# minyoungg/pix2latent

Measured on AMD Instinct MI355X. Metric: candidate-latent evals/sec (fwd+loss+bwd), BigGAN-256 pop=18, higher is better.
Workload: dtype f32 (fp32 tensors everywhere; convolutions >= 32x32 and the self-attention multiply on the 16-bit MFMA pipe with fp32-grade operand splits and fp32 accumulate: the 16x16 Winograd, direct and sub-pixel 3x3 kernels and the 1x1 kernels (4x4 layers included) on power-of-two scaled operands in 2 fp16 pie

## Files before the change

### include/p2l.h

```cpp
#ifndef P2L_H_
#define P2L_H_

#include <stddef.h>
#include <stdint.h>

#ifdef __cplusplus
extern "C" {
#endif

#define P2L_OK 0
#define P2L_EINVAL (-1)
#define P2L_ELAUNCH (-2)
#define P2L_EWS (-3)
#define P2L_EUNSUP (-4)

int p2l_version(void);
const char* p2l_strerror(int rc);
int p2l_last_hip_error(void);


enum { P2L_ACT_NONE = 0, P2L_ACT_RELU = 1, P2L_ACT_TANH = 2,
       P2L_ACT_LRELU_SQRT2 = 3  };
enum { P2L_POOL_NONE = 0, P2L_POOL_MAX = 1, P2L_POOL_SUM = 2 };
enum { P2L_PRO_NONE = 0, P2L_PRO_AFFINE_RELU = 1, P2L_PRO_AFFINE = 2 };
// ... 99 lines not shown

int p2l_pack_conv_weight(const float* w_oihw, int O, int I, int taps, int N_pad,
                         int K_pad, int transpose_flip, float* w_packed,
                         void* stream);

int p2l_pack_conv_weight_subpix(const float* w_oihw, int O, int I, int N_pad,
                                int K_pad, int transpose_flip, int mode,
                                float* w_packed, void* stream);

enum { P2L_WFMT_F32 = 0, P2L_WFMT_BF16X3 = 1, P2L_WFMT_BF16X3W = 2, P2L_WFMT_PW = 3,
       P2L_WFMT_BF16X3T = 4, P2L_WFMT_FLAG_PW = 0x10, P2L_WFMT_FLAG_THIN = 0x20,
       P2L_WFMT_FLAG_ATTN_GEMM = 0x40,
       P2L_WFMT_FLAG_NO_AMAX = 0x80
                                       };
int p2l_pack_conv_weight_bf3t(const float* w_oihw, int O, int I, int N_pad, int K_pad,
                              int transpose_flip, float* w_packed, void* stream);
int p2l_pack_conv_weight_pw(const float* w_oihw, int O, int I, int N_pad, int K_pad,
                            int transpose_flip, float* w_packed, void* stream);
size_t p2l_packed_weight_floats(int taps, int N_pad, int K_pad, int wfmt);
enum {
  P2L_FORM_AUTO = 0,
  P2L_FORM_NO_WINO = 1,
  P2L_FORM_WINO_ANY = 2,
  P2L_FORM_WINO_8X16 = 4,
  P2L_FORM_NO_PW = 8,
  P2L_FORM_NO_THIN = 16,
  P2L_FORM_WINO_BF3 = 32,
  P2L_FORM_WINO_H2_8X16 = 64,
  P2L_FORM_WINO_H2_16X16 = 128,
  P2L_FORM_NO_H2R = 256,
  P2L_FORM_H2R_SEQ_EPI = 512,
  P2L_FORM_NO_SP_SKIP = 1024,
  P2L_FORM_NO_SP_PAIR = 2048,
  P2L_FORM_SP_PAIR = 4096
};
int p2l_wino_split_factor(int H, int W, int Cin, int Cout);
int p2l_pack_conv_weight_bf3w(const float* w_oihw, int O, int I, int taps, int N_pad,
                              int K_pad, int transpose_flip, float* w_packed, void* stream);
int p2l_pack_conv_weight_bf3(const float* w_oihw, int O, int I, int taps, int N_pad,
                             int K_pad, int transpose_flip, float* w_packed, void* stream);
int p2l_pack_conv_weight_subpix_bf3(const float* w_oihw, int O, int I, int N_pad, int K_pad,
                                    int transpose_flip, int mode, float* w_packed,
                                    void* stream);
size_t p2l_packed_subpix_weight_floats(int N_pad, int K_pad, int wfmt);
int p2l_pack_conv_weight_subpix_h2(const float* w_oihw, int O, int I, int N_pad, int K_pad,
                                   int transpose_flip, int mode, float* w_packed, void* stream);

typedef struct P2LGemm {
  int32_t batch, M, N, K;
  int32_t lda, ldb, ldc;
  int64_t stride_a, stride_b, stride_c;
  int32_t a_kmajor, b_kmajor;
  float alpha;
  int32_t accumulate;
} P2LGemm;
int p2l_gemm(const P2LGemm* d, const float* A, const float* B, float* C,
             void* stream);
size_t p2l_gemm_ws_bytes(const P2LGemm* d);
int p2l_gemm_ws(const P2LGemm* d, const float* A, const float* B, float* C, void* ws,
                size_t ws_bytes, void* stream);

typedef struct P2LAttn {
  int32_t B, Nq, Nk, d, dv;
} P2LAttn;
int p2l_attn_supported(const P2LAttn* d);
size_t p2l_attn_fwd_ws_bytes(const P2LAttn* d);
int p2l_attn_fwd(const P2LAttn* d, const float* q, const float* k, const float* v, float* out,
                 float* lse, void* ws, size_t ws_bytes, void* stream);
// ... 384 lines not shown
```

### pix2latent_amd/_native.py

```python
import ctypes as C
import os

import torch

_HERE = os.path.dirname(os.path.abspath(__file__))
LIB_PATH = os.environ.get('P2L_LIB_PATH') or os.path.join(_HERE, 'libp2l_hip.so')

c_float_p = C.c_void_p


class P2LConv(C.Structure):
    _fields_ = [('B', C.c_int32), ('H', C.c_int32), ('W', C.c_int32),
                ('Cin', C.c_int32), ('Cout', C.c_int32), ('taps', C.c_int32),
                ('ups', C.c_int32), ('x_ld', C.c_int32), ('pro', C.c_int32),
                ('pro_bstride', C.c_int32), ('alpha', C.c_float), ('act', C.c_int32),
                ('pool', C.c_int32), ('y_ld', C.c_int32), ('yp_ld', C.c_int32),
                ('n_store', C.c_int32), ('res_ld', C.c_int32), ('res_ups', C.c_int32),
                ('mask_ld', C.c_int32), ('splitk', C.c_int32), ('ext', C.c_int32),
                ('wfmt', C.c_int32), ('form', C.c_int32), ('algo_flops', C.c_double),
                ('w_floats', C.c_int64)]


class P2LAmax(C.Structure):
    _fields_ = [('out', C.c_void_p), ('outp', C.c_void_p), ('in_', C.c_void_p), ('in_n', C.c_int32),
# ... 111 lines not shown
class P2LProfTotals(C.Structure):
    _fields_ = [('size', C.c_uint32), ('count', C.c_int32 * 2), ('reserved0', C.c_int32),
                ('flops', C.c_double * 2), ('ms', C.c_double * 2), ('bytes', C.c_double * 2),
                ('exec_flops', C.c_double * 2), ('mfma_flops', C.c_double * 2),
                ('write_bytes', C.c_double * 2),
                ('fam_count', C.c_int32 * 8), ('fam_ms', C.c_double * 8), ('fam_flops', C.c_double * 8),
                ('fam_mfma_flops', C.c_double * 8), ('fam_bytes', C.c_double * 8)]


PROF_FAMILIES = {0: 'other (exact-fp32 / bf16x3 direct, 8x16 Winograd)', 1: 'wino16s_conv_kernel<.., H2>',
                 2: 'conv_h2_kernel<9, ..>', 3: 'conv_h2_kernel<4, ..>', 4: 'conv_thinin/thinout_kernel',
                 5: 'pw_h2_kernel / pw_conv_kernel', 6: 'conv_h2r_kernel<..>'}


def prof_totals():
    t = P2LProfTotals()
    t.size = C.sizeof(P2LProfTotals)
    check(lib().p2l_prof_totals(C.byref(t)), 'p2l_prof_totals')
    return t


prof_end = prof_totals


ACT_NONE, ACT_RELU, ACT_TANH, ACT_LRELU_SQRT2 = 0, 1, 2, 3
WFMT_F32, WFMT_BF16X3, WFMT_BF16X3W, WFMT_PW, WFMT_BF16X3T = 0, 1, 2, 3, 4
WFMT_FLAG_PW, WFMT_FLAG_THIN, WFMT_FLAG_ATTN_GEMM, WFMT_FLAG_NO_AMAX = 0x10, 0x20, 0x40, 0x80
FORM_AUTO, FORM_NO_WINO, FORM_WINO_ANY, FORM_WINO_8X16, FORM_NO_PW, FORM_NO_THIN, FORM_WINO_BF3 = 0, 1, 2, 4, 8, 16, 32
FORM_WINO_H2_8X16, FORM_WINO_H2_16X16 = 64, 128
FORM_H2R_SEQ_EPI = 512
FORM_NO_SP_SKIP = 1024
FORM_NO_SP_PAIR = 2048
FORM_SP_PAIR = 4096
FORM_NO_H2R = 256


def default_wfmt():
    v = os.environ.get('P2L_CONV_WFMT', 'bf16x3').lower()
    if v in ('f32', 'fp32', '0'):
        return WFMT_F32
    if v in ('bf16x3-direct', 'bf3d', '1'):
        return WFMT_BF16X3
    if v in ('bf16x3', 'bf3', 'bf16x3w', '2'):
        return WFMT_BF16X3W
    raise ValueError('P2L_CONV_WFMT=%r (expected f32, bf16x3 or bf16x3-direct)' % v)


def default_thin():
    return os.environ.get('P2L_THIN', '1') != '0' and default_wfmt() != WFMT_F32


def default_attn_gemm():
    return os.environ.get('P2L_ATTN', '1') == '0'


def default_no_amax():
    return os.environ.get('P2L_AMAX', '1') == '0'


def default_pw():
    return os.environ.get('P2L_PW', '1') != '0' and default_wfmt() != WFMT_F32


def pack_conv_weight(src, taps, n_pad, k_pad, flip, wfmt, subpix_mode=None):
    L = lib()
    O, I = src.shape[0], src.shape[1]
# ... 9 lines not shown
    if subpix_mode is not None:
        dst = torch.empty(L.p2l_packed_subpix_weight_floats(n_pad, k_pad, wfmt), device=src.device,
                          dtype=torch.float32)
        fn = {WFMT_F32: L.p2l_pack_conv_weight_subpix,
              WFMT_BF16X3W: L.p2l_pack_conv_weight_subpix_h2}.get(wfmt, L.p2l_pack_conv_weight_subpix_bf3)
        check(fn(ptr(src), O, I, n_pad, k_pad, int(flip), int(subpix_mode), ptr(dst), stream()),
              'p2l_pack_conv_weight_subpix')
        return dst
    n = L.p2l_packed_weight_floats(taps, n_pad, k_pad, wfmt)
    dst = torch.empty(n, device=src.device, dtype=torch.float32)
    if wfmt == WFMT_BF16X3T:
        check(L.p2l_pack_conv_weight_bf3t(ptr(src), O, I, n_pad, k_pad, int(flip), ptr(dst), stream()),
              'p2l_pack_conv_weight_bf3t')
        return dst
    fn = {WFMT_F32: L.p2l_pack_conv_weight, WFMT_BF16X3: L.p2l_pack_conv_weight_bf3,
          WFMT_BF16X3W: L.p2l_pack_conv_weight_bf3w}[wfmt]
    check(fn(ptr(src), O, I, taps, n_pad, k_pad, int(flip), ptr(dst), stream()),
          'p2l_pack_conv_weight')
    return dst
def pack_gconv_weight(src, taps, n_pad, k_pad, flip):
    L = lib()
    src = src.detach().float().contiguous()
    dst = torch.empty(taps * n_pad * k_pad, device=src.device, dtype=torch.float32)
    check(L.p2l_pack_gconv_weight(ptr(src), src.shape[0], src.shape[1], taps, n_pad, k_pad, int(flip), ptr(dst),
                                  stream()), 'p2l_pack_gconv_weight')
    return dst


POOL_NONE, POOL_MAX, POOL_SUM = 0, 1, 2
PRO_NONE, PRO_AFFINE_RELU, PRO_AFFINE = 0, 1, 2

EXPORTS = [
    'p2l_version', 'p2l_strerror', 'p2l_last_hip_error',
    'p2l_conv_workspace_bytes', 'p2l_conv_amax_slots', 'p2l_selftest_amaxreg', 'p2l_conv_suggest_splitk', 'p2l_conv_fwd', 'p2l_conv_fwd_ex',
    'p2l_pack_conv_weight', 'p2l_pack_conv_weight_subpix', 'p2l_pack_conv_weight_bf3',
    'p2l_pack_conv_weight_bf3w', 'p2l_packed_weight_floats', 
    'p2l_pack_conv_weight_bf3t',
    'p2l_pack_conv_weight_pw', 'p2l_adam_step_dev',
    'p2l_attn_supported', 'p2l_attn_fwd_ws_bytes', 'p2l_attn_fwd', 'p2l_attn_bwd_dv_ws_bytes',
    'p2l_attn_bwd_dv', 'p2l_attn_bwd_qk_ws_bytes', 'p2l_attn_bwd_qk',
    'p2l_pack_conv_weight_subpix_bf3', 'p2l_pack_conv_weight_subpix_h2', 'p2l_packed_subpix_weight_floats', 'p2l_gemm', 'p2l_gemm_ws_bytes', 'p2l_gemm_ws', 'p2l_linear_fwd', 'p2l_linear_bwd',
    'p2l_cbn_fold_fwd', 'p2l_cbn_fold_bwd', 'p2l_affine_relu_bwd_nblk',
    'p2l_affine_relu_bwd', 'p2l_softmax_fwd', 'p2l_softmax_bwd', 'p2l_maxpool2_bwd', 'p2l_maxpool2_bwd_amax', 'p2l_maxpool2_bwd_amax_slots',
    'p2l_relu_mask', 'p2l_nchw3_to_nhwc16', 'p2l_nhwc16_to_nchw3', 'p2l_tanh_bwd16',
    'p2l_weight_sum', 'p2l_weight_map', 'p2l_l1_loss_nblk', 'p2l_l1_loss_fwd',
    'p2l_l1_loss_bwd', 'p2l_lpips_normalize', 'p2l_lpips_tap_nblk', 'p2l_lpips_tap_fwd',
    'p2l_lpips_tap_bwd', 'p2l_lpips_tap_pool_bwd', 'p2l_bilinear_adjoint', 'p2l_reduce_rows', 'p2l_adam_step',
    'p2l_clamp', 'p2l_affine_grid_sample', 'p2l_affine_grid_sample_bwd', 'p2l_affine_grid_sample_bwd_ws_bytes', 'p2l_vec_scale_div', 'p2l_concat2', 'p2l_split2',
    'p2l_biggan_ws_bytes', 'p2l_biggan_fwd', 'p2l_biggan_bwd', 'p2l_biggan_ws_lookup',
    'p2l_loss_cache_floats', 'p2l_projloss_ws_bytes', 'p2l_projloss_ws_lookup', 'p2l_projloss_prepare',
    'p2l_projloss_fwd', 'p2l_projloss_bwd', 'p2l_mfma_probe', 'p2l_prof_begin', 'p2l_prof_totals', 'p2l_prof_step', 'p2l_prof_dump', 'p2l_wino_split_factor', 'p2l_linear_fwd_ld', 'p2l_linear_bwd_ld', 'p2l_scale_bwd',
    'p2l_sg2_pixelnorm_fwd', 'p2l_sg2_pixelnorm_bwd', 'p2l_sg2_bias_lrelu_fwd', 'p2l_sg2_lrelu_bwd',
    'p2l_sg2_demod_fwd', 'p2l_sg2_demod_bwd', 'p2l_sg2_blur_fwd', 'p2l_sg2_act_bwd_nblk',
    'p2l_sg2_styled_act_bwd', 'p2l_sg2_blur_bwd', 'p2l_sg2_rgb_up_fwd', 'p2l_sg2_rgb_up_bwd',
    'p2l_sg2_clamp16_fwd', 'p2l_sg2_clamp16_bwd', 'p2l_broadcast_rows', 'p2l_add_inplace',
    'p2l_sg2_ws_bytes', 'p2l_sg2_ws_lookup', 'p2l_sg2_synthesis_fwd', 'p2l_sg2_synthesis_bwd', 'p2l_sg2_mapping_fwd',
    'p2l_sg2_mapping_bwd', 'p2l_conv_arb_fusable', 'p2l_conv_arb_nblk',
    'p2l_conv_dgrad_arb', 'p2l_conv_arb_split_fusable', 'p2l_conv_arb_nblk_ws',
    'p2l_conv_dgrad_arb_ws', 'p2l_arb_finish', 'p2l_arb_defer_begin', 'p2l_arb_defer_flush',
    'p2l_arb_defer_cancel',
    'p2l_gconv_fwd', 'p2l_maxpool3s2_fwd', 'p2l_maxpool3s2_bwd', 'p2l_conv1_dgrad',
    'p2l_alex_cache_floats', 'p2l_alexloss_ws_bytes', 'p2l_alexloss_prepare', 'p2l_alexloss_fwd',
    'p2l_alexloss_bwd',
    'p2l_pack_gconv_weight', 'p2l_sqz_cache_floats', 'p2l_sqzloss_ws_bytes', 'p2l_sqzloss_prepare', 'p2l_sqzloss_fwd',
    'p2l_sqzloss_bwd', 'p2l_sqzloss_ws_lookup',
    'p2l_sg2_blur_fwd_amax', 'p2l_sg2_styled_act_bwd_amax', 'p2l_sg2_blur_bwd_amax', 'p2l_sg2_noise_relayout',
    'p2l_sg2_rows_defer_begin', 'p2l_sg2_rows_defer_flush', 'p2l_sg2_rows_defer_cancel',
# ... 90 lines not shown
```

### pix2latent_amd/csrc/p2l_conv.hip

```cpp
#include "p2l_conv_k.h"

#include <cstdlib>
#include <cstring>
#include <cstddef>
#include <array>
#include <atomic>
#include <cstdio>
#include <mutex>
#include <string>
#include <vector>

using namespace p2lconv;

namespace {

struct ConvProf {
  std::atomic<bool> on{false};
  int n = 0;
  std::vector<hipEvent_t> ev;
  std::vector<double> flops;
  std::vector<double> xflops;
  std::vector<int> nprod;
  std::vector<double> bytes;
  std::vector<double> wbytes;
// ... 964 lines not shown
static bool direct_h2r(const P2LConv* d) {
  if ((d->form & P2L_FORM_NO_H2R) || !direct_h2(d)) return false;
  if (!p2l_h2r_shape(d->taps, d->ups, d->H, d->W, d->Cin, d->Cout, d->x_ld)) return false;
  return d->H * d->W >= 128 && direct_split(d) <= 1;
}


static int subpix_bwd_split(const P2LConv* d) {
  if (d->ups != 3 || !d->ext || !direct_h2(d)) return 1;
  ConvK k{};
  if (choose_tile(d, k) != P2L_OK || k.partial) return 1;
  const long hw = (long)(d->H >> 1) * (d->W >> 1);
  int s = p2f((long)d->Cin * 16 / 128);
  const int g = p2f(524288L / (hw * d->Cout > 0 ? hw * d->Cout : 1));
  if (g < s) s = g;
  const int cap = hw >= 256 ? 4 : 8;
  if (s > cap) s = cap;
  const int nchunks = 4 * (d->Cin / 16);
  while (s > 1 && nchunks / s < 8) s >>= 1;
  return s <= 2 ? 1 : s;
}

extern "C" int p2l_conv_suggest_splitk(const P2LConv* d) {
  ConvK k{};
  if (d && d->ups == 3 && d->ext) return subpix_bwd_split(d);
  if (!d || d->ups >= 2) return 1;
  if (choose_tile(d, k) == P2L_OK && wino_split(d) > 1 && !(d->form & P2L_FORM_WINO_ANY) &&
      (d->H / 8) * (d->W / 16) * (d->Cout / 64) < 64)
    return wino_split(d);
  if (choose_tile(d, k) != P2L_OK || k.partial || wino_shape(d) || pw_any(d)) return 1;
  return direct_split(d);
}

static bool wino_h2(const P2LConv* d) {
  return wino_shape(d) && d->H % 16 == 0 && d->W % 16 == 0 &&
         !(d->form & (P2L_FORM_WINO_8X16 | P2L_FORM_WINO_BF3));
}
static int effective_splitk(const P2LConv* d);
static bool finish_v4_ok(const P2LConv* d) {
#ifdef P2L_AB_SCALAR_FINISH
  return false;
#endif
  return d->n_store % 4 == 0 && d->Cout % 4 == 0 && d->y_ld % 4 == 0 && d->yp_ld % 4 == 0 &&
         d->res_ld % 4 == 0 && d->mask_ld % 4 == 0;
}
extern "C" int p2l_conv_amax_slots(const P2LConv* d) {
  if (!d) return 0;
  if (wino_shape(d)) {
    if (d->H % 16 || d->W % 16 || (d->form & P2L_FORM_WINO_8X16)) return 0;
    if (d->splitk > 1 && wino_split(d) == d->splitk) {
      const int per_image = (d->H / 2) * (d->W / 2) * (d->n_store / 4);
      return (per_image % 64 == 0 && d->n_store % 4 == 0) ? per_image / 64 : 0;
    }
    return (d->H / 16) * (d->W / 16) * (d->Cout / 64) * 8;
  }
  if (d->ups == 3 && effective_splitk(d) > 1) return 0;
  if (effective_splitk(d) > 1) {
    const int per_image = (d->H / 2) * (d->W / 2) * (finish_v4_ok(d) ? d->n_store / 4 : d->n_store);
    return (per_image % 64 == 0) ? per_image / 64 : 0;
  }
  ConvK k{};
  if (choose_tile(d, k) != P2L_OK || k.tb_log != 0 || k.partial) return 0;
  const int tm = thin_shape(d);
  if (tm >= 0) {
    const bool geom = k.tw_log == 4 && k.th_log == 3;
    return (tm == 1 && geom) ? k.tiles_x * k.tiles_y * 4 : 0;
// ... 719 lines not shown
```

### pix2latent_amd/csrc/p2l_conv_k.h

```cpp
#pragma once
#include "p2l_common.h"

namespace p2lconv {

struct ConvK {
  const float* x;
  const float* w;
  const float* bias;
  const float* pro_s;
  const float* pro_t;
  const float* res;
  const float* mask;
  float* y;
  float* yp;
  float* ws;
  int B, H, W, Cin, Cout;
  int x_ld, y_ld, yp_ld, res_ld, mask_ld, n_store;
  int pro_bstride;
  float alpha;
  int act, pool, res_ups, ups;
  int nchunks, chunks_per_split, splitk;
  int tw_log, th_log, tb_log;
  int tiles_x_log, tiles_y_log;
  int n_mtiles, n_ntiles;
// ... 343 lines not shown
      if (k.amax_out != nullptr) k.amax_out[slot] = m;
      if (k.amax_outp != nullptr) k.amax_outp[slot] = mp;
    }
  }
}


}

int p2l_pw_launch(const p2lconv::ConvK& k, int pro, hipStream_t st);

size_t p2l_thin_weight_floats(int N_pad, int K_pad);
int p2l_thin_mode(int N_pad, int K_pad);
int p2l_thin_pack(const float* w_oihw, int O, int I, int N_pad, int K_pad, int flip, float* dst,
                  hipStream_t st);
int p2l_thinin_launch(const p2lconv::ConvK& k, int pro, hipStream_t st);
int p2l_thinout_launch(const p2lconv::ConvK& k, int pro, hipStream_t st);

extern "C" size_t p2l_wino_weight_floats(int N_pad, int K_pad);
extern "C" int p2l_wino_weight_ok(int N_pad, int K_pad);
extern "C" int p2l_wino_split_factor(int H, int W, int Cin, int Cout);
extern "C" size_t p2l_wino_h2_weight_floats(int N_pad, int K_pad);
extern "C" size_t p2l_pw_h2_weight_floats(int N_pad, int K_pad);
int p2l_pw_pack_h2(const float* w_oihw, int O, int I, int N_pad, int K_pad, int flip, float* dst, hipStream_t st);
int p2l_wino_pack(const float* w_oihw, int O, int I, int N_pad, int K_pad, int transpose_flip,
                  float* dst, hipStream_t st);
int p2l_wino_launch(const p2lconv::ConvK& k, int pro, hipStream_t st);
int p2l_amax_launch(const p2lconv::ConvK& k, int pro, hipStream_t st);

size_t p2l_h2_weight_floats(int N_pad, int K_pad, int subpix);
int p2l_h2_pack(const float* w_oihw, int O, int I, int N_pad, int K_pad, int flip, int mode, float* dst,
                hipStream_t st);
int p2l_h2_launch(const p2lconv::ConvK& k, int pro, int taps, int bn, bool small, hipStream_t st);

bool p2l_h2r_shape(int taps, int ups, int H, int W, int Cin, int Cout, int x_ld);
bool p2l_h2r_takes(const p2lconv::ConvK& k);
int p2l_h2r_launch(const p2lconv::ConvK& k, int pro, hipStream_t st);
```

### pix2latent_amd/csrc/p2l_h2.hip

```cpp
#include "p2l_conv_k.h"

#include <atomic>
#include <type_traits>

using namespace p2lconv;

namespace {

#ifndef P2L_H2_ABL
#define P2L_H2_ABL 0
#endif

__device__ __forceinline__ int h2c(int c, int row) { return c ^ ((row >> 2) & 3) ^ (((row >> 1) & 1) << 1); }

#define P2L_WAIT(VM, LGKM) __builtin_amdgcn_s_waitcnt(((VM) & 15) | (7 << 4) | ((LGKM) << 8) | (((VM) >> 4) << 14))

template <int TAPS, int BN, int A_ITERS, int PRO, bool SKIP = false>
__global__ __launch_bounds__(256, 2) void conv_h2_kernel(const ConvK k) {
  constexpr bool SUBPIX = (TAPS == 4 || TAPS == 8);
  constexpr int NP = (TAPS == 8) ? 2 : 1;
  constexpr int NT = BN / 32;
  constexpr int B_ITEMS = TAPS * BN * 4;
  constexpr int B_ITERS = (B_ITEMS + 255) / 256;
  constexpr int SL = SUBPIX ? 16 : TAPS;
  constexpr int T0 = (TAPS == 4) ? 2 : 4;
  constexpr int NU = TAPS * NT, U0 = T0 * NT;
  constexpr int H0 = U0 * 128;
  static_assert(H0 % 256 == 0, "half 0 must be whole DMA instructions");
  constexpr int NH1_MIN = (B_ITEMS - H0) / 256;
  constexpr bool S_UNI = (A_ITERS == 3);
  constexpr int S_ITERS = S_UNI ? 1 : A_ITERS;
  constexpr int NA_LD = A_ITERS + ((PRO != P2L_PRO_NONE) ? 2 * S_ITERS : 0);

  extern __shared__ __attribute__((aligned(16))) float smem[];

  const int tid = threadIdx.x;
  const int lane = tid & 63, wave = tid >> 6;
  const int l31 = lane & 31, lhi = lane >> 5;

  const int TW = 1 << k.tw_log, TH = 1 << k.th_log, TB = 1 << k.tb_log;
  const int HW_ = TW + 2, HH_ = TH + 2;
  const int HP = k.hp;
  const int a_rows = TB * HH_ * HW_;
  const int a_rows_lds = TB * HH_ * HP;
  char* As = reinterpret_cast<char*>(smem);
  char* Bs = As + (size_t)a_rows_lds * 64;
  const int main_floats = max(a_rows_lds * 16 + TAPS * BN * 16, 4 * 32 * (BN + 4));
  float* scl = smem + main_floats;

  const int swz = xcd_remap(blockIdx.x, gridDim.x);
  const int mt = swz / k.n_ntiles, nt = swz - mt * k.n_ntiles;
  const int tiles_per_image = k.tiles_x * k.tiles_y;
  const int bt = mt / tiles_per_image;
  const int tile_in_image = mt - bt * tiles_per_image;
  const int ty = tile_in_image / k.tiles_x, tx = tile_in_image - ty * k.tiles_x;
  const int n0 = nt * BN;
  const int y0 = ty << k.th_log, x0 = tx << k.tw_log, b0 = bt << k.tb_log;

  const bool sp_fwd = SUBPIX && (TAPS == 8 || k.sp_mode == 1);
  const bool sp_bwd = (TAPS == 4) && k.sp_mode == 2;
  const int z = sp_fwd ? 0 : blockIdx.y;
  const int ph_y = sp_fwd ? (TAPS == 8 ? (int)blockIdx.y : (int)(blockIdx.y >> 1)) : 0;
  const int ph_x = (sp_fwd && TAPS == 4) ? (int)(blockIdx.y & 1) : 0;
  const int c_begin = z * k.chunks_per_split;
  const int c_end = min(k.nchunks, c_begin + k.chunks_per_split);

  const int av = tid & 3;
  int a_goff[A_ITERS];
  int a_soff[A_ITERS];
  int a_row[A_ITERS];
  float a_xs[S_ITERS];
  int a_tb[S_ITERS];
  unsigned a_valid = 0;
#pragma unroll
  for (int it = 0; it < A_ITERS; ++it) {
    const int p = (tid + 256 * it) >> 2;
    a_goff[it] = 0;
    a_soff[it] = 0;
    a_row[it] = -1;
    if (it < S_ITERS) { a_xs[it] = 1.f; a_tb[it] = 0; }
// ... 30 lines not shown
        a_extra = ((cls >> 1) * k.ibW + (cls & 1)) * k.x_ld;
      } else {
        wslab = (ph_y * 2 + ph_x) * 4;
      }
    }
  };
  int b_goff[B_ITERS];
#pragma unroll
  for (int it = 0; it < B_ITERS; ++it) {
    const int jj = tid + 256 * it;
    const int u = jj >> 7, within = jj & 127;
    const int tap = u / NT, j = u - tap * NT;
    b_goff[it] = ((j * SL + tap) * 32) * 16 + within * 4;
  }
  auto dma_b = [&](int c, auto half_c) {
    constexpr int half = decltype(half_c)::value;
    int cc, wslab, a_extra;
    geom(c, cc, wslab, a_extra);
    const float* base = k.w + ((((size_t)cc * (k.Cout >> 5) + (n0 >> 5)) * SL + wslab) * 32) * 16;
#pragma unroll
    for (int it = 0; it < B_ITERS; ++it) {
      if ((half == 0 && 256 * it >= H0) || (half == 1 && 256 * (it + 1) <= H0)) continue;
      const int jj = tid + 256 * it;
      if (jj < B_ITEMS) {
        const float* src = base + b_goff[it];
        if (SUBPIX && SKIP) {
          unsigned lv;
          if (TAPS == 8) { const unsigned my = ph_y ? 0x3u : 0xFu; lv = my | ((my & 0x5u) << 4); }
          else if (sp_fwd) lv = (ph_y ? 0x3u : 0xFu) & (ph_x ? 0x5u : 0xFu);
          else { const int cls = c / k.sp_ncc; lv = ((cls >> 1) ? 0xCu : 0xFu) & ((cls & 1) ? 0xAu : 0xFu); }
          const int tap = (jj >> 7) / NT;
          if (!((lv >> tap) & 1u)) src = base;
        }
        const unsigned lds_wave_base = __builtin_amdgcn_readfirstlane(
            (unsigned)(size_t)(__attribute__((address_space(3))) char*)(Bs + (size_t)(jj - lane) * 16));
        asm volatile("s_mov_b32 m0, %1\n\ts_nop 0\n\tglobal_load_lds_dwordx4 %0, off"
                     :: "v"(src), "s"(lds_wave_base) : "memory");
      }
    }
  };
  auto load_a = [&](int c) {
    int cc, wslab, a_extra;
    geom(c, cc, wslab, a_extra);
#pragma unroll
    for (int it = 0; it < A_ITERS; ++it) {
      xr[it] = *reinterpret_cast<const f32x4*>(k.x + (size_t)(a_goff[it] + a_extra) + cc * 16);
      if (PRO != P2L_PRO_NONE && it < S_ITERS) {
        const int so = S_UNI ? s_uni : a_soff[it];
        sr[it] = *reinterpret_cast<const f32x4*>(k.pro_s + so + cc * 16);
        tr[it] = *reinterpret_cast<const f32x4*>(k.pro_t + so + cc * 16);
      }
    }
  };
  auto write_a = [&]() {
#pragma unroll
    for (int it = 0; it < A_ITERS; ++it) {
      if (a_row[it] >= 0) {
        f32x4 v = xr[it];
        if (PRO != P2L_PRO_NONE) {
          v = v * sr[S_UNI ? 0 : it] + tr[S_UNI ? 0 : it];
          if (PRO == P2L_PRO_AFFINE_RELU) {
            v.x = fmaxf(v.x, 0.f); v.y = fmaxf(v.y, 0.f);
            v.z = fmaxf(v.z, 0.f); v.w = fmaxf(v.w, 0.f);
          }
        }
        if (!((a_valid >> it) & 1u)) v = f32x4{0.f, 0.f, 0.f, 0.f};
        v = v * a_xs[S_UNI ? 0 : it];
        const h16x4 h = __builtin_convertvector(v, h16x4);
        const f32x4 w = __builtin_convertvector(h, f32x4);
        const h16x4 m = __builtin_convertvector(v - w, h16x4);
        const int row = a_row[it];
        char* rb = As + row * 64 + (av & 1) * 8;
        *reinterpret_cast<h16x4*>(rb + h2c(av >> 1, row) * 16) = h;
        *reinterpret_cast<h16x4*>(rb + h2c(2 + (av >> 1), row) * 16) = m;
      }
    }
  };

  int a_row0;
  {
    const int i = wave * 32 + l31;
    const int Q = i >> 2, s = i & 3;
    const int qx = Q & ((TW >> 1) - 1);
    const int qy = (Q >> (k.tw_log - 1)) & ((TH >> 1) - 1);
    const int tb = Q >> (k.tw_log + k.th_log - 2);
    a_row0 = (tb * HH_ + 2 * qy + (s >> 1)) * HP + 2 * qx + (s & 1);
  }
  const int b_h = l31 * 64 + h2c(lhi, l31) * 16, b_m = l31 * 64 + h2c(2 + lhi, l31) * 16;

  f32x16 acc[NP * NT];
#pragma unroll
  for (int j = 0; j < NP * NT; ++j)
#pragma unroll
    for (int r = 0; r < 16; ++r) acc[j][r] = 0.f;

  using H0c = std::integral_constant<int, 0>;
  using H1c = std::integral_constant<int, 1>;
  if (c_begin < c_end) {
    dma_b(c_begin, H0c{});
    dma_b(c_begin, H1c{});
    load_a(c_begin);
  }
  {
    float sw, inv_w;
    h2_scales(__builtin_amdgcn_readfirstlane(k.w_tail[0]), sw, inv_w);
    const int step = (TB == 1) ? 256 : 64, me = (TB == 1) ? tid : lane;
    for (int t = (TB == 1) ? 0 : wave; t < TB; t += 4) {
      const int b = b0 + t;
      float a = 0.f, ms = 0.f, mtt = 0.f;
      if (b < k.B) {
        if (k.amax_in != nullptr) {
          for (int i = me; i < k.amax_in_n; i += step) a = fmaxf(a, k.amax_in[(size_t)b * k.amax_in_n + i]);
          if (PRO != P2L_PRO_NONE && !k.amax_in_applied) {
            const f32x4* ps = reinterpret_cast<const f32x4*>(k.pro_s + (size_t)b * k.pro_bstride);
            const f32x4* pt = reinterpret_cast<const f32x4*>(k.pro_t + (size_t)b * k.pro_bstride);
            for (int c = me; c < (k.Cin >> 2); c += step) {
              const f32x4 s4 = ps[c], t4 = pt[c];
              ms = fmaxf(fmaxf(ms, fmaxf(fabsf(s4.x), fabsf(s4.y))), fmaxf(fabsf(s4.z), fabsf(s4.w)));
              mtt = fmaxf(fmaxf(mtt, fmaxf(fabsf(t4.x), fabsf(t4.y))), fmaxf(fabsf(t4.z), fabsf(t4.w)));
            }
          }
        } else if (me < 64) {
          a = k.amax[b * 64 + me];
        }
      }
#pragma unroll
      for (int o = 1; o < 64; o <<= 1) {
        a = fmaxf(a, __shfl_xor(a, o, 64));
        if (PRO != P2L_PRO_NONE) { ms = fmaxf(ms, __shfl_xor(ms, o, 64)); mtt = fmaxf(mtt, __shfl_xor(mtt, o, 64)); }
      }
      if (TB == 1) {
        if (lane == 0) { smem[wave * 4] = a; smem[wave * 4 + 1] = ms; smem[wave * 4 + 2] = mtt; }
        __syncthreads();
        a = fmaxf(fmaxf(smem[0], smem[4]), fmaxf(smem[8], smem[12]));
        ms = fmaxf(fmaxf(smem[1], smem[5]), fmaxf(smem[9], smem[13]));
        mtt = fmaxf(fmaxf(smem[2], smem[6]), fmaxf(smem[10], smem[14]));
      }
      if (PRO != P2L_PRO_NONE && k.amax_in != nullptr) a = (k.amax_in_applied ? a : ms * a + mtt) * 1.001f;
      float xs, inv_x;
      h2_scales(__builtin_bit_cast(unsigned, a), xs, inv_x);
      if ((TB == 1) ? (tid == 0) : (lane == 0)) { scl[2 * t] = xs; scl[2 * t + 1] = inv_x * inv_w; }
      if (TB == 1) break;
    }
    __syncthreads();
  }

  if (S_UNI) {
    a_xs[0] = scl[0];
  } else {
#pragma unroll
    for (int it = 0; it < S_ITERS; ++it) a_xs[it] = scl[2 * a_tb[it]];
  }
  if (c_begin < c_end) {
    write_a();
    __builtin_amdgcn_sched_barrier(0);
    if (c_begin + 1 < c_end) load_a(c_begin + 1);
  }
  __builtin_amdgcn_sched_barrier(0);
  P2L_WAIT(NA_LD, 0);
  __builtin_amdgcn_s_barrier();

  for (int c = c_begin; c < c_end; ++c) {
    const bool more = (c + 1 < c_end);
    int win_row = 0;
    if (SUBPIX) {
      int oy = ph_y, ox = ph_x;
      if (sp_bwd) {
        const int cls = c / k.sp_ncc;
        oy = 1 - (cls >> 1);
        ox = 1 - (cls & 1);
      }
      win_row = oy * HP + ox;
    }
    unsigned live = 0xFFu;
    if (SUBPIX && SKIP) {
      if (TAPS == 8) {
        const unsigned my = ph_y ? 0x3u : 0xFu;
        live = my | ((my & 0x5u) << 4);
      } else if (sp_fwd) {
        live = (ph_y ? 0x3u : 0xFu) & (ph_x ? 0x5u : 0xFu);
      } else {
        const int cls = c / k.sp_ncc;
        live = ((cls >> 1) ? 0xCu : 0xFu) & ((cls & 1) ? 0xAu : 0xFu);
      }
    }
    h16x8 af[2][2], bq[2][2];
    auto lda = [&](int tap, h16x8 (&a)[2]) {
      const int dy = (TAPS == 9) ? tap / 3 : ((tap & 3) >> 1);
      const int dx = (TAPS == 9) ? tap - dy * 3 : (tap & 1);
      const int arow = a_row0 + win_row + dy * HP + dx + ((TAPS == 8) ? (tap >> 2) : 0);
      const char* ar = As + arow * 64;
      a[0] = *reinterpret_cast<const h16x8*>(ar + h2c(lhi, arow) * 16);
      a[1] = *reinterpret_cast<const h16x8*>(ar + h2c(2 + lhi, arow) * 16);
    };
    auto ldb = [&](int u, h16x8 (&b)[2]) {
      const char* br = Bs + u * (32 * 64);
      b[0] = *reinterpret_cast<const h16x8*>(br + b_h);
      b[1] = *reinterpret_cast<const h16x8*>(br + b_m);
    };
    lda(0, af[0]);
    ldb(0, bq[0]);
#pragma unroll
    for (int u = 0; u < NU; ++u) {
      const int tap = u / NT, j = u - tap * NT;
      if (u == U0) {
        if (more) P2L_WAIT(NA_LD, 0); else P2L_WAIT(0, 0);
        if (!(P2L_H2_ABL & 16)) __builtin_amdgcn_s_barrier();
        if (more && !(P2L_H2_ABL & 4)) dma_b(c + 1, H0c{});
        if (j == 0) lda(tap, af[tap & 1]);
        ldb(u, bq[u & 1]);
      }
      if (u + 1 < NU && u + 1 != U0) {
        const int tn = (u + 1) / NT, jn = (u + 1) - tn * NT;
        if (!(SUBPIX && SKIP) || ((live >> tn) & 1u)) {
          if (jn == 0) lda(tn, af[tn & 1]);
          ldb(u + 1, bq[(u + 1) & 1]);
        }
      }
      __builtin_amdgcn_sched_barrier(0);
      const h16x8 (&a)[2] = af[tap & 1];
      const h16x8 (&b)[2] = bq[u & 1];
      if (SUBPIX && SKIP && !((live >> tap) & 1u)) continue;
      const int ja = (TAPS == 8) ? (tap >> 2) * NT + j : j;
      if (!(P2L_H2_ABL & 8)) {
      acc[ja] = __builtin_amdgcn_mfma_f32_32x32x16_f16(a[1], b[0], acc[ja], 0, 0, 0);
      acc[ja] = __builtin_amdgcn_mfma_f32_32x32x16_f16(a[0], b[1], acc[ja], 0, 0, 0);
      acc[ja] = __builtin_amdgcn_mfma_f32_32x32x16_f16(a[0], b[0], acc[ja], 0, 0, 0);
      } else { acc[ja][0] += (float)a[0][0] * (float)b[0][0]; }
      __builtin_amdgcn_sched_barrier(0);
    }
    P2L_WAIT(63, 0);
    if (!(P2L_H2_ABL & 16)) __builtin_amdgcn_s_barrier();
    if (more) {
      if (!(P2L_H2_ABL & 1)) write_a();
      __builtin_amdgcn_sched_barrier(0);
      const bool more2 = (c + 2 < c_end);
      if (!(P2L_H2_ABL & 4)) dma_b(c + 1, H1c{});
      __builtin_amdgcn_sched_barrier(0);
      if (more2 && !(P2L_H2_ABL & 2)) load_a(c + 2);
      __builtin_amdgcn_sched_barrier(0);
      if (more2) P2L_WAIT(NA_LD + NH1_MIN, 0); else P2L_WAIT(NH1_MIN, 0);
    } else {
      P2L_WAIT(63, 0);
    }
    if (!(P2L_H2_ABL & 16)) __builtin_amdgcn_s_barrier();
  }

  if (S_UNI) {
    const float os = scl[1];
#pragma unroll
    for (int j = 0; j < NP * NT; ++j)
#pragma unroll
      for (int r = 0; r < 16; ++r) acc[j][r] *= os;
  } else {
#pragma unroll
    for (int g = 0; g < 4; ++g) {
      const int Q = wave * 8 + 2 * g + lhi;
      const float os = scl[2 * (Q >> (k.tw_log + k.th_log - 2)) + 1];
#pragma unroll
      for (int j = 0; j < NP * NT; ++j)
#pragma unroll
        for (int s = 0; s < 4; ++s) acc[j][4 * g + s] *= os;
    }
  }

  if (k.splitk > 1) {
    const size_t mtot = (size_t)k.B * k.H * k.W;
#pragma unroll
    for (int g = 0; g < 4; ++g) {
      const int Q = wave * 8 + 2 * g + lhi;
      const int qx = Q & ((TW >> 1) - 1);
      const int qy = (Q >> (k.tw_log - 1)) & ((TH >> 1) - 1);
      const int b = b0 + (Q >> (k.tw_log + k.th_log - 2));
      if (b >= k.B) continue;
      const size_t pix0 = ((size_t)b * k.H + y0 + 2 * qy) * k.W + x0 + 2 * qx;
#pragma unroll
      for (int j = 0; j < NT; ++j) {
        float* wp = k.ws + ((size_t)z * mtot + pix0) * k.Cout + n0 + j * 32 + l31;
        wp[0] = acc[j][g * 4 + 0];
        wp[k.Cout] = acc[j][g * 4 + 1];
        wp[(size_t)k.W * k.Cout] = acc[j][g * 4 + 2];
        wp[(size_t)(k.W + 1) * k.Cout] = acc[j][g * 4 + 3];
      }
    }
  } else {
    __syncthreads();
    if (!(P2L_H2_ABL & 32) || acc[0][0] == 12345.678f) {
      if (TAPS == 8) {
#pragma unroll
        for (int p = 0; p < NP; ++p) {
          if (p) __syncthreads();
          epilogue_vec<NT>(k, reinterpret_cast<f32x16 (&)[NT]>(acc[p * NT]), smem, wave, lane, b0, y0, x0, n0,
                           tile_in_image, 1, ph_y, p);
        }
      } else {
        epilogue_vec<NT>(k, reinterpret_cast<f32x16 (&)[NT]>(acc[0]), smem, wave, lane, b0, y0, x0, n0, tile_in_image,
                         sp_fwd ? 1 : 0, ph_y, ph_x);
      }
    }
// ... 67 lines not shown
                        : src[((size_t)n * I + c) * 9 + dy * 3 + dx];
      }
    }
    const float x = v * scale;
    const _Float16 h = (_Float16)x;
    ph[e] = h; pm[e] = (_Float16)(x - (float)h);
  }
  char* rb = reinterpret_cast<char*>(dst) +
             ((((size_t)q * (N_pad >> 5) + tile) * n_slabs + slab) * 32 + row) * 64;
  *reinterpret_cast<h16x8*>(rb + h2c(kh, row) * 16) = ph;
  *reinterpret_cast<h16x8*>(rb + h2c(2 + kh, row) * 16) = pm;
}

}

size_t p2l_h2_weight_floats(int N_pad, int K_pad, int subpix) {
  return (size_t)N_pad * K_pad * (subpix ? 16 : 9) + 4;
}
int p2l_h2_pack(const float* w_oihw, int O, int I, int N_pad, int K_pad, int flip, int mode, float* dst,
                hipStream_t st) {
  const int n_slabs = mode < 0 ? 9 : 16;
  unsigned* tail = reinterpret_cast<unsigned*>(dst + (size_t)N_pad * K_pad * n_slabs);
  if (hipMemsetAsync(tail, 0, 16, st) != hipSuccess) return P2L_ELAUNCH;
  const size_t nw = (size_t)O * I * 9;
  hipLaunchKernelGGL(h2_wmax_kernel, dim3((unsigned)(cdiv(nw, 256) < 256 ? cdiv(nw, 256) : 256)), dim3(256), 0, st,
                     w_oihw, nw, tail);
  if (mode >= 0) hipLaunchKernelGGL(h2_tail_x4_kernel, dim3(1), dim3(1), 0, st, tail);
  const size_t total = (size_t)(K_pad >> 4) * (N_pad >> 5) * n_slabs * 32 * 2;
  hipLaunchKernelGGL(h2_pack_kernel, dim3(cdiv(total, 256)), dim3(256), 0, st, w_oihw, dst, O, I, N_pad, K_pad,
                     flip, mode, tail);
  return p2l_check_launch();
}

size_t p2l_h2_lds_bytes(const ConvK& k, int taps, int bn) {
  const int TB = 1 << k.tb_log, TH = 1 << k.th_log;
  const int a_rows_lds = TB * (TH + 2) * k.hp;
  int main_floats = a_rows_lds * 16 + taps * bn * 16;
  const int epi = 4 * 32 * (bn + 4);
  if (epi > main_floats) main_floats = epi;
  return (size_t)(main_floats + 2 * TB + 16) * sizeof(float);
}

int p2l_h2_launch(const ConvK& k, int pro, int taps, int bn, bool small, hipStream_t st) {
  dim3 grid(k.n_mtiles * k.n_ntiles, taps == 8 ? 2 : (taps == 4 && k.sp_mode == 1) ? 4 : k.splitk), block(256);
  const size_t lds = p2l_h2_lds_bytes(k, taps, bn);
#define P2L_H2L(TAPS, BNV, AIT, PROV)                                                         \
  do {                                                                                        \
    if ((TAPS == 4 || TAPS == 8) && k.sp_skip) P2L_H2K(TAPS, BNV, AIT, PROV, (TAPS == 4 || TAPS == 8)); \
    else P2L_H2K(TAPS, BNV, AIT, PROV, false);                                                \
  } while (0)
#define P2L_H2K(TAPS, BNV, AIT, PROV, SKIPV)                                                  \
  do {                                                                                        \
    auto kfn = conv_h2_kernel<TAPS, BNV, AIT, PROV, SKIPV>;                                   \
    static std::atomic<bool> attr_set{false};                                                 \
    if (!attr_set) {                                                                          \
      (void)hipFuncSetAttribute((const void*)kfn, hipFuncAttributeMaxDynamicSharedMemorySize, \
                                160 * 1024);                                                  \
      attr_set = true;                                                                        \
    }                                                                                         \
    hipLaunchKernelGGL(kfn, grid, block, lds, st, k);                                         \
  } while (0)
#define P2L_H2P(TAPS, BNV, AIT)                                                               \
  do {                                                                                        \
    if (pro == P2L_PRO_NONE) P2L_H2L(TAPS, BNV, AIT, P2L_PRO_NONE);                           \
    else if (pro == P2L_PRO_AFFINE_RELU) P2L_H2L(TAPS, BNV, AIT, P2L_PRO_AFFINE_RELU);        \
    else P2L_H2L(TAPS, BNV, AIT, P2L_PRO_AFFINE);                                             \
  } while (0)
  if (taps == 9) {
    if (bn == 64) { if (small) P2L_H2P(9, 64, 3); else P2L_H2P(9, 64, 5); }
    else          { if (small) P2L_H2P(9, 32, 3); else P2L_H2P(9, 32, 5); }
  } else if (taps == 8) {
    if (bn == 64) { if (small) P2L_H2P(8, 64, 3); else P2L_H2P(8, 64, 5); }
    else          { if (small) P2L_H2P(8, 32, 3); else P2L_H2P(8, 32, 5); }
  } else {
    if (bn == 64) { if (small) P2L_H2P(4, 64, 3); else P2L_H2P(4, 64, 5); }
    else          { if (small) P2L_H2P(4, 32, 3); else P2L_H2P(4, 32, 5); }
  }
#undef P2L_H2P
#undef P2L_H2L
#undef P2L_H2K
  return p2l_check_launch();
}
```

Before: 1215.

## Add multi-slot B-tile streaming pipeline to split-K direct h2 conv kernel

Adds a streaming variant of the direct 3x3 fp16-split conv kernel for split-K launches. It keeps up to four weight (B) tiles in flight in an LDS ring buffer instead of double-buffering half-tiles inside the tap loop, which removes the mid-loop wait and barrier. The ring depth is sized to fit in 160KB of LDS. The larger LDS footprint can lower occupancy, and the epilogue always takes the split-K path. A host query function exposing the LDS size and depth is also added.

```diff
diff --git a/include/p2l.h b/include/p2l.h
--- a/include/p2l.h
+++ b/include/p2l.h
@@ -155,8 +155,10 @@
   P2L_FORM_H2R_SEQ_EPI = 512,
   P2L_FORM_NO_SP_SKIP = 1024,
   P2L_FORM_NO_SP_PAIR = 2048,
-  P2L_FORM_SP_PAIR = 4096
+  P2L_FORM_SP_PAIR = 4096,
+  P2L_FORM_NO_H2_STREAM = 8192
 };
+int p2l_conv_h2_lds_bytes(const P2LConv* d, int32_t info[4]);
 int p2l_wino_split_factor(int H, int W, int Cin, int Cout);
 int p2l_pack_conv_weight_bf3w(const float* w_oihw, int O, int I, int taps, int N_pad,
                               int K_pad, int transpose_flip, float* w_packed, void* stream);
diff --git a/pix2latent_amd/_native.py b/pix2latent_amd/_native.py
--- a/pix2latent_amd/_native.py
+++ b/pix2latent_amd/_native.py
@@ -167,6 +167,7 @@
 FORM_NO_SP_SKIP = 1024
 FORM_NO_SP_PAIR = 2048
 FORM_SP_PAIR = 4096
+FORM_NO_H2_STREAM = 8192
 FORM_NO_H2R = 256
 
 
@@ -242,7 +243,7 @@
 
 EXPORTS = [
     'p2l_version', 'p2l_strerror', 'p2l_last_hip_error',
-    'p2l_conv_workspace_bytes', 'p2l_conv_amax_slots', 'p2l_selftest_amaxreg', 'p2l_conv_suggest_splitk', 'p2l_conv_fwd', 'p2l_conv_fwd_ex',
+    'p2l_conv_workspace_bytes', 'p2l_conv_amax_slots', 'p2l_selftest_amaxreg', 'p2l_conv_suggest_splitk', 'p2l_conv_h2_lds_bytes', 'p2l_conv_fwd', 'p2l_conv_fwd_ex',
     'p2l_pack_conv_weight', 'p2l_pack_conv_weight_subpix', 'p2l_pack_conv_weight_bf3',
     'p2l_pack_conv_weight_bf3w', 'p2l_packed_weight_floats', 
     'p2l_pack_conv_weight_bf3t',
diff --git a/pix2latent_amd/csrc/p2l_conv.hip b/pix2latent_amd/csrc/p2l_conv.hip
--- a/pix2latent_amd/csrc/p2l_conv.hip
+++ b/pix2latent_amd/csrc/p2l_conv.hip
@@ -1020,6 +1020,28 @@
   return direct_split(d);
 }
 
+extern "C" int p2l_conv_h2_lds_bytes(const P2LConv* d, int32_t info[4]) {
+  if (!d || d->taps != 9 || d->ups != 0 || d->Cin % 16 || d->Cout % 32 || !direct_h2(d) || thin_shape(d) >= 0) return 0;
+  ConvK k{};
+  k.form = d->form;
+  if (choose_tile(d, k) != P2L_OK) return 0;
+  k.hp = halo_pitch_h2(1 << k.tw_log);
+  k.nchunks = d->Cin / 16;
+  k.splitk = d->splitk < 1 ? 1 : (d->splitk > k.nchunks ? k.nchunks : d->splitk);
+  k.chunks_per_split = cdiv(k.nchunks, k.splitk);
+  k.splitk = cdiv(k.nchunks, k.chunks_per_split);
+  if (direct_h2r(d) && k.splitk == 1 && !k.partial && k.tb_log == 0) return 0;
+  const int bn = direct_h2r(d) ? 64 : choose_bn(d, k.n_mtiles);
+  const int nd = p2l_h2_stream_depth(k, 9, bn);
+  if (info) {
+    info[0] = nd ? nd : 1;
+    info[1] = 9 * bn * 64;
+    info[2] = (1 << k.tb_log) * ((1 << k.th_log) + 2) * k.hp * 64;
+    info[3] = k.chunks_per_split;
+  }
+  return (int)p2l_h2_lds_bytes(k, 9, bn);
+}
+
 static bool wino_h2(const P2LConv* d) {
   return wino_shape(d) && d->H % 16 == 0 && d->W % 16 == 0 &&
          !(d->form & (P2L_FORM_WINO_8X16 | P2L_FORM_WINO_BF3));
diff --git a/pix2latent_amd/csrc/p2l_conv_k.h b/pix2latent_amd/csrc/p2l_conv_k.h
--- a/pix2latent_amd/csrc/p2l_conv_k.h
+++ b/pix2latent_amd/csrc/p2l_conv_k.h
@@ -399,6 +399,8 @@
 int p2l_h2_pack(const float* w_oihw, int O, int I, int N_pad, int K_pad, int flip, int mode, float* dst,
                 hipStream_t st);
 int p2l_h2_launch(const p2lconv::ConvK& k, int pro, int taps, int bn, bool small, hipStream_t st);
+int p2l_h2_stream_depth(const p2lconv::ConvK& k, int taps, int bn);
+size_t p2l_h2_lds_bytes(const p2lconv::ConvK& k, int taps, int bn);
 
 bool p2l_h2r_shape(int taps, int ups, int H, int W, int Cin, int Cout, int x_ld);
 bool p2l_h2r_takes(const p2lconv::ConvK& k);
diff --git a/pix2latent_amd/csrc/p2l_h2.hip b/pix2latent_amd/csrc/p2l_h2.hip
--- a/pix2latent_amd/csrc/p2l_h2.hip
+++ b/pix2latent_amd/csrc/p2l_h2.hip
@@ -15,7 +15,16 @@
 
 #define P2L_WAIT(VM, LGKM) __builtin_amdgcn_s_waitcnt(((VM) & 15) | (7 << 4) | ((LGKM) << 8) | (((VM) >> 4) << 14))
 
-template <int TAPS, int BN, int A_ITERS, int PRO, bool SKIP = false>
+#ifndef P2L_H2_STREAM_MAX
+#define P2L_H2_STREAM_MAX 4
+#endif
+__host__ __device__ inline int h2_stream_depth(int a_rows_lds, int tb, int bn, int chunks_per_split) {
+  const int fit = (160 * 1024 - a_rows_lds * 64 - (2 * tb + 16) * 4) / (9 * bn * 64);
+  const int want = chunks_per_split < P2L_H2_STREAM_MAX ? chunks_per_split : P2L_H2_STREAM_MAX;
+  return want < fit ? want : fit;
+}
+
+template <int TAPS, int BN, int A_ITERS, int PRO, bool SKIP = false, bool STREAM = false>
 __global__ __launch_bounds__(256, 2) void conv_h2_kernel(const ConvK k) {
   constexpr bool SUBPIX = (TAPS == 4 || TAPS == 8);
   constexpr int NP = (TAPS == 8) ? 2 : 1;
@@ -28,6 +37,9 @@
   constexpr int H0 = U0 * 128;
   static_assert(H0 % 256 == 0, "half 0 must be whole DMA instructions");
   constexpr int NH1_MIN = (B_ITEMS - H0) / 256;
+  constexpr int NB_MIN = B_ITEMS / 256;
+  constexpr int TILE_BYTES = TAPS * BN * 64;
+  static_assert(!STREAM || (TAPS == 9 && !SKIP), "the streaming form is the stride-1 split-K one");
   constexpr bool S_UNI = (A_ITERS == 3);
   constexpr int S_ITERS = S_UNI ? 1 : A_ITERS;
   constexpr int NA_LD = A_ITERS + ((PRO != P2L_PRO_NONE) ? 2 * S_ITERS : 0);
@@ -45,7 +57,11 @@
   const int a_rows_lds = TB * HH_ * HP;
   char* As = reinterpret_cast<char*>(smem);
   char* Bs = As + (size_t)a_rows_lds * 64;
-  const int main_floats = max(a_rows_lds * 16 + TAPS * BN * 16, 4 * 32 * (BN + 4));
+  [[maybe_unused]] const int ND = STREAM ? h2_stream_depth(a_rows_lds, TB, BN, k.chunks_per_split) : 1;
+  [[maybe_unused]] char* Bw = Bs;
+  [[maybe_unused]] const char* Br = Bs;
+  const int main_floats = STREAM ? a_rows_lds * 16 + ND * TAPS * BN * 16
+                                 : max(a_rows_lds * 16 + TAPS * BN * 16, 4 * 32 * (BN + 4));
   float* scl = smem + main_floats;
 
   const int swz = xcd_remap(blockIdx.x, gridDim.x);
@@ -142,8 +158,10 @@
           const int tap = (jj >> 7) / NT;
           if (!((lv >> tap) & 1u)) src = base;
         }
+        char* bdst = Bs;
+        if constexpr (STREAM) bdst = Bw;
         const unsigned lds_wave_base = __builtin_amdgcn_readfirstlane(
-            (unsigned)(size_t)(__attribute__((address_space(3))) char*)(Bs + (size_t)(jj - lane) * 16));
+            (unsigned)(size_t)(__attribute__((address_space(3))) char*)(bdst + (size_t)(jj - lane) * 16));
         asm volatile("s_mov_b32 m0, %1\n\ts_nop 0\n\tglobal_load_lds_dwordx4 %0, off"
                      :: "v"(src), "s"(lds_wave_base) : "memory");
       }
@@ -206,7 +224,14 @@
 
   using H0c = std::integral_constant<int, 0>;
   using H1c = std::integral_constant<int, 1>;
-  if (c_begin < c_end) {
+  if constexpr (STREAM) {
+    for (int i = 0; i < ND && c_begin + i < c_end; ++i) {
+      Bw = Bs + i * TILE_BYTES;
+      dma_b(c_begin + i, H0c{});
+      dma_b(c_begin + i, H1c{});
+    }
+    if (c_begin < c_end) load_a(c_begin);
+  } else if (c_begin < c_end) {
     dma_b(c_begin, H0c{});
     dma_b(c_begin, H1c{});
     load_a(c_begin);
@@ -267,11 +292,17 @@
     if (c_begin + 1 < c_end) load_a(c_begin + 1);
   }
   __builtin_amdgcn_sched_barrier(0);
-  P2L_WAIT(NA_LD, 0);
+  if constexpr (STREAM) {
+    if (c_begin + 1 < c_end) P2L_WAIT(NA_LD, 0); else P2L_WAIT(0, 0);
+  } else {
+    P2L_WAIT(NA_LD, 0);
+  }
   __builtin_amdgcn_s_barrier();
 
+  [[maybe_unused]] int slot = 0;
   for (int c = c_begin; c < c_end; ++c) {
     const bool more = (c + 1 < c_end);
+    if constexpr (STREAM) Br = Bs + slot * TILE_BYTES;
     int win_row = 0;
     if (SUBPIX) {
       int oy = ph_y, ox = ph_x;
@@ -305,6 +336,7 @@
     };
     auto ldb = [&](int u, h16x8 (&b)[2]) {
       const char* br = Bs + u * (32 * 64);
+      if constexpr (STREAM) br = Br + u * (32 * 64);
       b[0] = *reinterpret_cast<const h16x8*>(br + b_h);
       b[1] = *reinterpret_cast<const h16x8*>(br + b_m);
     };
@@ -313,14 +345,14 @@
 #pragma unroll
     for (int u = 0; u < NU; ++u) {
       const int tap = u / NT, j = u - tap * NT;
-      if (u == U0) {
+      if (!STREAM && u == U0) {
         if (more) P2L_WAIT(NA_LD, 0); else P2L_WAIT(0, 0);
         if (!(P2L_H2_ABL & 16)) __builtin_amdgcn_s_barrier();
         if (more && !(P2L_H2_ABL & 4)) dma_b(c + 1, H0c{});
         if (j == 0) lda(tap, af[tap & 1]);
         ldb(u, bq[u & 1]);
       }
-      if (u + 1 < NU && u + 1 != U0) {
+      if (u + 1 < NU && (STREAM || u + 1 != U0)) {
         const int tn = (u + 1) / NT, jn = (u + 1) - tn * NT;
         if (!(SUBPIX && SKIP) || ((live >> tn) & 1u)) {
           if (jn == 0) lda(tn, af[tn & 1]);
@@ -341,6 +373,26 @@
     }
     P2L_WAIT(63, 0);
     if (!(P2L_H2_ABL & 16)) __builtin_amdgcn_s_barrier();
+    if constexpr (STREAM) {
+      if (more) {
+        write_a();
+        __builtin_amdgcn_sched_barrier(0);
+        const bool refill = (c + ND < c_end), more2 = (c + 2 < c_end);
+        if (refill) {
+          Bw = Bs + slot * TILE_BYTES;
+          dma_b(c + ND, H0c{});
+          dma_b(c + ND, H1c{});
+        }
+        __builtin_amdgcn_sched_barrier(0);
+        if (more2) load_a(c + 2);
+        __builtin_amdgcn_sched_barrier(0);
+        if (refill) { if (more2) P2L_WAIT(NA_LD + NB_MIN, 0); else P2L_WAIT(NB_MIN, 0); }
+        else        { if (more2) P2L_WAIT(NA_LD, 0); else P2L_WAIT(0, 0); }
+      } else {
+        P2L_WAIT(63, 0);
+      }
+      slot = (slot + 1 == ND) ? 0 : slot + 1;
+    } else
     if (more) {
       if (!(P2L_H2_ABL & 1)) write_a();
       __builtin_amdgcn_sched_barrier(0);
@@ -374,7 +426,7 @@
     }
   }
 
-  if (k.splitk > 1) {
+  if (STREAM || k.splitk > 1) {
     const size_t mtot = (size_t)k.B * k.H * k.W;
 #pragma unroll
     for (int g = 0; g < 4; ++g) {
@@ -508,18 +560,27 @@
   return p2l_check_launch();
 }
 
+int p2l_h2_stream_depth(const ConvK& k, int taps, int bn) {
+  if (taps != 9 || k.splitk <= 1 || (k.form & P2L_FORM_NO_H2_STREAM)) return 0;
+  const int TB = 1 << k.tb_log, TH = 1 << k.th_log;
+  const int nd = h2_stream_depth(TB * (TH + 2) * k.hp, TB, bn, k.chunks_per_split);
+  return nd >= 2 ? nd : 0;
+}
+
 size_t p2l_h2_lds_bytes(const ConvK& k, int taps, int bn) {
   const int TB = 1 << k.tb_log, TH = 1 << k.th_log;
   const int a_rows_lds = TB * (TH + 2) * k.hp;
-  int main_floats = a_rows_lds * 16 + taps * bn * 16;
+  const int nd = p2l_h2_stream_depth(k, taps, bn);
+  int main_floats = a_rows_lds * 16 + (nd ? nd : 1) * taps * bn * 16;
   const int epi = 4 * 32 * (bn + 4);
-  if (epi > main_floats) main_floats = epi;
+  if (!nd && epi > main_floats) main_floats = epi;
   return (size_t)(main_floats + 2 * TB + 16) * sizeof(float);
 }
 
 int p2l_h2_launch(const ConvK& k, int pro, int taps, int bn, bool small, hipStream_t st) {
   dim3 grid(k.n_mtiles * k.n_ntiles, taps == 8 ? 2 : (taps == 4 && k.sp_mode == 1) ? 4 : k.splitk), block(256);
   const size_t lds = p2l_h2_lds_bytes(k, taps, bn);
+  const bool stream = p2l_h2_stream_depth(k, taps, bn) > 0;
 #define P2L_H2L(TAPS, BNV, AIT, PROV)                                                         \
   do {                                                                                        \
     if ((TAPS == 4 || TAPS == 8) && k.sp_skip) P2L_H2K(TAPS, BNV, AIT, PROV, (TAPS == 4 || TAPS == 8)); \
@@ -542,7 +603,30 @@
     else if (pro == P2L_PRO_AFFINE_RELU) P2L_H2L(TAPS, BNV, AIT, P2L_PRO_AFFINE_RELU);        \
     else P2L_H2L(TAPS, BNV, AIT, P2L_PRO_AFFINE);                                             \
   } while (0)
-  if (taps == 9) {
+#define P2L_H2S(BNV, AIT, PROV)                                                               \
+  do {                                                                                        \
+    auto kfn = conv_h2_kernel<9, BNV, AIT, PROV, false, true>;                                \
+    static std::atomic<unsigned long long> attr_devs{0};                                      \
+    int dev = -1;                                                                             \
+    if (hipGetDevice(&dev) != hipSuccess) return P2L_ELAUNCH;                                 \
+    if (dev < 0 || dev >= 64 || !((attr_devs.load() >> dev) & 1ull)) {                        \
+      if (hipFuncSetAttribute((const void*)kfn, hipFuncAttributeMaxDynamicSharedMemorySize,   \
+                              160 * 1024) != hipSuccess) return P2L_ELAUNCH;                  \
+      if (dev >= 0 && dev < 64) attr_devs.fetch_or(1ull << dev);                              \
+    }                                                                                         \
+    hipLaunchKernelGGL(kfn, grid, block, lds, st, k);                                         \
+  } while (0)
+#define P2L_H2SP(BNV, AIT)                                                                    \
+  do {                                                                                        \
+    if (pro == P2L_PRO_NONE) P2L_H2S(BNV, AIT, P2L_PRO_NONE);                                 \
+    else if (pro == P2L_PRO_AFFINE_RELU) P2L_H2S(BNV, AIT, P2L_PRO_AFFINE_RELU);              \
+    else P2L_H2S(BNV, AIT, P2L_PRO_AFFINE);                                                   \
+  } while (0)
+  if (taps == 9 && stream) {
+    if (lds > 160 * 1024) return P2L_EUNSUP;
+    if (bn == 64) { if (small) P2L_H2SP(64, 3); else P2L_H2SP(64, 5); }
+    else          { if (small) P2L_H2SP(32, 3); else P2L_H2SP(32, 5); }
+  } else if (taps == 9) {
     if (bn == 64) { if (small) P2L_H2P(9, 64, 3); else P2L_H2P(9, 64, 5); }
     else          { if (small) P2L_H2P(9, 32, 3); else P2L_H2P(9, 32, 5); }
   } else if (taps == 8) {
@@ -552,6 +636,8 @@
     if (bn == 64) { if (small) P2L_H2P(4, 64, 3); else P2L_H2P(4, 64, 5); }
     else          { if (small) P2L_H2P(4, 32, 3); else P2L_H2P(4, 32, 5); }
   }
+#undef P2L_H2SP
+#undef P2L_H2S
 #undef P2L_H2P
 #undef P2L_H2L
 #undef P2L_H2K
```

New measurement: 1195. -1.6%, worse.
